# Ghundi/fluid_simulation

Hardware: AMD Instinct MI355X
Metric: cells_steps_per_sec (higher is better)
Workload: dtype f32

## Files before the change

### fluid_simulation_amd/csrc/kernels.hip

```cpp
#include <hip/hip_runtime.h>
#include "kernels.h"
#include "kernels_dev.h"
#include <type_traits>

namespace fs {

template <class T, int RY>
struct PlaneIn {
    T core[RY][4];
    T hb[4], ht[4];
    T eL[RY], eR[RY];
};
template <class T, int RY>
struct AuxIn {
    T rhs[RY][4];
    unsigned fl[RY];
};

template <class T, int RY, int ABL, bool PUSH>
__global__ __launch_bounds__(256) void jacobi_sweep_kernel(GridDesc g, SlabCtx sc, const T* __restrict__ src,
                                                            const T* __restrict__ rhs, T* __restrict__ dst,
                                                            const uint8_t* __restrict__ flags, int b, T a, T inv_c,
                                                            int z_first, int z_last, int zc_len, int z_stride, int nxw,
                                                            int nybg, int nblk, PeerPush pp)
// ... 774 lines not shown
    }
}


template <class T>
__global__ void bounds_faces_kernel(GridDesc g, SlabCtx sc, T* q, int b)
{
    const int W = g.W, H = g.H, D = g.D;
    const long nx = (long)H * D, ny = (long)W * D, nz = (long)W * H;
    for (long t = blockIdx.x * (long)blockDim.x + threadIdx.x; t < nx + ny + nz; t += (long)gridDim.x * blockDim.x) {
        if (t < nx) {
            int y = 1 + (int)(t % H), z = 1 + (int)(t / H);
            T in = q[cell(g, 1, y, z)];
            q[cell(g, 0, y, z)] = (b == 1) ? -in : in;
            q[cell(g, W + 1, y, z)] = q[cell(g, W, y, z)];
        } else if (t < nx + ny) {
            long u = t - nx;
            int x = 1 + (int)(u % W), z = 1 + (int)(u / W);
            T lo = q[cell(g, x, 1, z)], hi = q[cell(g, x, H, z)];
            q[cell(g, x, 0, z)] = (b == 2) ? -lo : lo;
            q[cell(g, x, H + 1, z)] = (b == 2) ? -hi : hi;
        } else {
            long u = t - nx - ny;
            int x = 1 + (int)(u % W), y = 1 + (int)(u / W);
            if (sc.lo_wall) {
                T lo = q[cell(g, x, y, 1)];
                q[cell(g, x, y, 0)] = (b == 3) ? -lo : lo;
            }
            if (sc.hi_wall) {
                T hi = q[cell(g, x, y, D)];
                q[cell(g, x, y, D + 1)] = (b == 3) ? -hi : hi;
            }
        }
    }
}

template <class T>
__global__ void bounds_zero_kernel(GridDesc g, T* q, const uint8_t* flags, int b)
{
    const int x = 1 + blockIdx.x * blockDim.x + threadIdx.x;
    const int y = 1 + blockIdx.y * blockDim.y + threadIdx.y;
    const int z = 1 + blockIdx.z;
    if (x > g.W || y > g.H) return;
    const unsigned zero_bits = (b == 0) ? F_SOLID : (F_SOLID | F_NEAR);
    long c = cell(g, x, y, z);
    if (flags[c] & zero_bits) q[c] = (T)0;
}

static inline dim3 cell_grid(const GridDesc& g) { return dim3((g.W + 63) / 64, (g.H + 3) / 4, g.D); }
static inline dim3 cell_block() { return dim3(64, 4, 1); }

template <class T>
void launch_set_bounds(hipStream_t st, const GridDesc& g, const SlabCtx& sc, T* q, const uint8_t* flags, int b)
{
    long faces = (long)g.H * g.D + (long)g.W * g.D + (long)g.W * g.H;
    int nb = (int)((faces + 255) / 256);
    if (nb > 4096) nb = 4096;
    hipLaunchKernelGGL((bounds_faces_kernel<T>), dim3(nb), dim3(256), 0, st, g, sc, q, b);
    hipLaunchKernelGGL((bounds_zero_kernel<T>), cell_grid(g), cell_block(), 0, st, g, q, flags, b);
}
template void launch_set_bounds<float>(hipStream_t, const GridDesc&, const SlabCtx&, float*, const uint8_t*, int);
template void launch_set_bounds<double>(hipStream_t, const GridDesc&, const SlabCtx&, double*, const uint8_t*, int);


template <class T, bool STORE_P>
__global__ __launch_bounds__(256) void divergence_kernel(GridDesc g, SlabCtx sc, const T* __restrict__ vx,
                                                          const T* __restrict__ vy, const T* __restrict__ vz,
                                                          T* __restrict__ dv, T* __restrict__ p,
                                                          const uint8_t* __restrict__ flags, T mhalf_h)
{
    const int x = 1 + blockIdx.x * blockDim.x + threadIdx.x;
    const int y = 1 + blockIdx.y * blockDim.y + threadIdx.y;
    const int z = 1 + blockIdx.z;
    if (x > g.W || y > g.H) return;
    const long c = cell(g, x, y, z);
    const unsigned f = flags[c];
    T d = (T)0;
    if (!(f & F_SOLID)) {
        T acc = (T)0;
        if (f & F_XP) acc += vx[c + 1];
        if (f & F_XM) acc -= vx[c - 1];
        if (f & F_YP) acc += vy[c + g.sy];
        if (f & F_YM) acc -= vy[c - g.sy];
        if (f & F_ZP) acc += vz[c + g.sz];
        if (f & F_ZM) acc -= vz[c - g.sz];
        d = mhalf_h * acc;
    }
    dv[c] = d;
    write_face_ghosts(g, sc, dv, c, x, y, z, d, 0);
    if constexpr (STORE_P) {
        p[c] = (T)0;
        write_face_ghosts(g, sc, p, c, x, y, z, (T)0, 0);
    }
}

template <class T>
void launch_divergence(hipStream_t st, const SweepTune& tune, const GridDesc& g, const SlabCtx& sc, const T* vx, const T* vy,
                       const T* vz, T* div, T* p, const uint8_t* flags, T mhalf_h, bool store_p)
{
    if (tune.project_cell) {
        if (store_p)
            hipLaunchKernelGGL((divergence_kernel<T, true>), cell_grid(g), cell_block(), 0, st, g, sc, vx, vy, vz, div, p, flags,
                               mhalf_h);
        else
            hipLaunchKernelGGL((divergence_kernel<T, false>), cell_grid(g), cell_block(), 0, st, g, sc, vx, vy, vz, div, p, flags,
                               mhalf_h);
        return;
    }
    constexpr int RY = 2;
    const MarchLaunch m = march_launch(g, RY);
    if (store_p)
        hipLaunchKernelGGL((divergence_march_kernel<T, RY, true>), dim3(m.nblk), dim3(256), 0, st, g, sc, vx, vy, vz, div, p, flags,
                           mhalf_h, m.zc_len, m.nxw, m.nybg, m.nblk);
    else
        hipLaunchKernelGGL((divergence_march_kernel<T, RY, false>), dim3(m.nblk), dim3(256), 0, st, g, sc, vx, vy, vz, div, p, flags,
                           mhalf_h, m.zc_len, m.nxw, m.nybg, m.nblk);
}
template void launch_divergence<float>(hipStream_t, const SweepTune&, const GridDesc&, const SlabCtx&, const float*,
                                       const float*, const float*, float*, float*, const uint8_t*, float, bool);
template void launch_divergence<double>(hipStream_t, const SweepTune&, const GridDesc&, const SlabCtx&, const double*,
                                        const double*, const double*, double*, double*, const uint8_t*, double, bool);

template <class T>
__device__ __forceinline__ T one_sided_grad(bool fp, bool fm, T pp, T pc, T pm, T h, T two_h)
{
    if (fp && fm) return (pp - pm) / two_h;
    if (fp) return (pp - pc) / h;
    if (fm) return (pc - pm) / h;
    return (T)0;
}

template <class T>
__global__ __launch_bounds__(256) void gradient_kernel(GridDesc g, SlabCtx sc, const T* __restrict__ p,
                                                        T* __restrict__ vx, T* __restrict__ vy, T* __restrict__ vz,
                                                        const uint8_t* __restrict__ flags, T h, T two_h)
{
    const int x = 1 + blockIdx.x * blockDim.x + threadIdx.x;
    const int y = 1 + blockIdx.y * blockDim.y + threadIdx.y;
    const int z = 1 + blockIdx.z;
    if (x > g.W || y > g.H) return;
    const long c = cell(g, x, y, z);
    const unsigned f = flags[c];
    T ux = vx[c], uy = vy[c], uz = vz[c];
    if (!(f & F_SOLID)) {
        const T pc = p[c];
        ux -= one_sided_grad<T>(f & F_XP, f & F_XM, p[c + 1], pc, p[c - 1], h, two_h);
        uy -= one_sided_grad<T>(f & F_YP, f & F_YM, p[c + g.sy], pc, p[c - g.sy], h, two_h);
        uz -= one_sided_grad<T>(f & F_ZP, f & F_ZM, p[c + g.sz], pc, p[c - g.sz], h, two_h);
    }
    const bool kill = (f & (F_SOLID | F_NEAR)) != 0;
    vx[c] = kill ? (T)0 : ux;
    vy[c] = kill ? (T)0 : uy;
    vz[c] = kill ? (T)0 : uz;
    write_face_ghosts(g, sc, vx, c, x, y, z, ux, 1);
    write_face_ghosts(g, sc, vy, c, x, y, z, uy, 2);
    write_face_ghosts(g, sc, vz, c, x, y, z, uz, 3);
}

template <class T>
void launch_gradient(hipStream_t st, const SweepTune& tune, const GridDesc& g, const SlabCtx& sc, const T* p, T* vx, T* vy,
                     T* vz, const uint8_t* flags, T h, T two_h)
{
    if (tune.project_cell) {
        hipLaunchKernelGGL((gradient_kernel<T>), cell_grid(g), cell_block(), 0, st, g, sc, p, vx, vy, vz, flags, h, two_h);
        return;
    }
    constexpr int RY = 2;
    const MarchLaunch m = march_launch(g, RY);
    hipLaunchKernelGGL((gradient_march_kernel<T, RY>), dim3(m.nblk), dim3(256), 0, st, g, sc, p, vx, vy, vz, flags, h, two_h,
                       m.zc_len, m.nxw, m.nybg, m.nblk);
}
template void launch_gradient<float>(hipStream_t, const SweepTune&, const GridDesc&, const SlabCtx&, const float*, float*,
                                     float*, float*, const uint8_t*, float, float);
template void launch_gradient<double>(hipStream_t, const SweepTune&, const GridDesc&, const SlabCtx&, const double*,
                                      double*, double*, double*, const uint8_t*, double, double);

template <class T>
__device__ __forceinline__ T clamp_ref(T v, T lo, T hi) { return (v < lo) ? lo : ((hi < v) ? hi : v); }

typedef float pair_f __attribute__((ext_vector_type(2), aligned(4)));
typedef double pair_d __attribute__((ext_vector_type(2), aligned(8)));
template <class T> struct PairOf;
template <> struct PairOf<float> { using type = pair_f; };
template <> struct PairOf<double> { using type = pair_d; };
template <class T>
__device__ __forceinline__ typename PairOf<T>::type ld_pair(const T* p) { return *reinterpret_cast<const typename PairOf<T>::type*>(p); }

template <class T>
__device__ __forceinline__ T back_trace_tab(const GridDesc& g, const SlabCtx& sc, const T* __restrict__ src, long zshift,
                                            const T* __restrict__ tab, int x, int y, int z, T ux, T uy, T uz, T kx, T ky, T kz);

template <class T, bool TAB>
__global__ __launch_bounds__(256) void advect_kernel(GridDesc g, SlabCtx sc, int b, T* __restrict__ field,
                                                      const T* __restrict__ prev, const T* vx, const T* vy,
                                                      const T* vz, const uint8_t* __restrict__ flags, T kx, T ky, T kz,
                                                      long prev_zshift, const T* __restrict__ tab)
{
    const int x = 1 + blockIdx.x * blockDim.x + threadIdx.x;
    const int y = 1 + blockIdx.y * blockDim.y + __builtin_amdgcn_readfirstlane(threadIdx.y);
    const int z = 1 + blockIdx.z;
    if (x > g.W || y > g.H) return;
    const long c = cell(g, x, y, z);
    const unsigned f = flags[c];
    const T one = (T)1, half = (T)0.5;
    T u = (T)0;
    if (!(f & F_SOLID)) {
        T ux, uy, uz;
        if (b == 0) {
            ux = vx[c]; uy = vy[c]; uz = vz[c];
        } else {
            const T own = prev[c + prev_zshift];
            ux = (b == 1) ? own : vx[c];
            uy = (b == 2) ? own : vy[c];
            uz = (b == 3) ? own : vz[c];
        }
        if constexpr (TAB) {
            u = back_trace_tab<T>(g, sc, prev, prev_zshift, tab, x, y, z, ux, uy, uz, kx, ky, kz);
        } else {
        const int zg = z + sc.zoff;
        T px = clamp_ref<T>((T)x - kx * ux, half, (T)g.W + half);
        T py = clamp_ref<T>((T)y - ky * uy, half, (T)g.H + half);
        T pz = clamp_ref<T>((T)zg - kz * uz, half, (T)sc.Dglobal + half);
        const int x0 = (int)floor(px), y0 = (int)floor(py), z0 = (int)floor(pz);
        const T tx = px - (T)x0, ty = py - (T)y0, tz = pz - (T)z0;
        const T* s = prev + prev_zshift + cell(g, x0, y0, z0 - sc.zoff);
        const auto q00 = ld_pair(s), q01 = ld_pair(s + g.sz), q10 = ld_pair(s + g.sy), q11 = ld_pair(s + g.sy + g.sz);
        const T a00 = q00.x * (one - tx) + q00.y * tx;
        const T a01 = q01.x * (one - tx) + q01.y * tx;
        const T a10 = q10.x * (one - tx) + q10.y * tx;
        const T a11 = q11.x * (one - tx) + q11.y * tx;
        const T b0 = a00 * (one - ty) + a10 * ty;
        const T b1 = a01 * (one - ty) + a11 * ty;
        u = b0 * (one - tz) + b1 * tz;
        }
    }
    const bool kill = (b != 0) && (f & F_NEAR);
    field[c] = kill ? (T)0 : u;
    write_face_ghosts(g, sc, field, c, x, y, z, u, b);
}

template <class T>
__device__ __forceinline__ T back_trace(const GridDesc& g, const SlabCtx& sc, const T* __restrict__ src, long zshift,
                                        int x, int y, int z, T ux, T uy, T uz, T kx, T ky, T kz)
{
    const T one = (T)1, half = (T)0.5;
    T px = clamp_ref<T>((T)x - kx * ux, half, (T)g.W + half);
    T py = clamp_ref<T>((T)y - ky * uy, half, (T)g.H + half);
    T pz = clamp_ref<T>((T)(z + sc.zoff) - kz * uz, half, (T)sc.Dglobal + half);
    const int x0 = (int)floor(px), y0 = (int)floor(py), z0 = (int)floor(pz);
    const T tx = px - (T)x0, ty = py - (T)y0, tz = pz - (T)z0;
    const T* s = src + zshift + cell(g, x0, y0, z0 - sc.zoff);
    const auto q00 = ld_pair(s), q01 = ld_pair(s + g.sz), q10 = ld_pair(s + g.sy), q11 = ld_pair(s + g.sy + g.sz);
    const T a00 = q00.x * (one - tx) + q00.y * tx;
    const T a01 = q01.x * (one - tx) + q01.y * tx;
    const T a10 = q10.x * (one - tx) + q10.y * tx;
    const T a11 = q11.x * (one - tx) + q11.y * tx;
    const T b0 = a00 * (one - ty) + a10 * ty;
    const T b1 = a01 * (one - ty) + a11 * ty;
    return b0 * (one - tz) + b1 * tz;
}

template <class T, bool TAB>
__global__ __launch_bounds__(256) void advect_velocity_kernel(GridDesc g, SlabCtx sc, T* __restrict__ vx,
                                                               T* __restrict__ vy, T* __restrict__ vz,
                                                               const T* __restrict__ px, const T* __restrict__ py,
                                                               const T* __restrict__ pz,
                                                               const uint8_t* __restrict__ flags, T kx, T ky, T kz,
                                                               long zshift, const T* __restrict__ tab)
{
    const int x = 1 + blockIdx.x * blockDim.x + threadIdx.x;
    const int y = 1 + blockIdx.y * blockDim.y + __builtin_amdgcn_readfirstlane(threadIdx.y);
    const int z = 1 + blockIdx.z;
    if (x > g.W || y > g.H) return;
    const long c = cell(g, x, y, z);
    const unsigned f = flags[c];
    const bool near = (f & F_NEAR) != 0;
    T nx = (T)0, ny = (T)0, nz = (T)0;
    T sx = (T)0, sy = (T)0;
    if (!(f & F_SOLID)) {
        const T oy = vy[c], oz = vz[c];
        if constexpr (TAB) {
            const long plane2 = 2 * (long)(g.H + 2) * (g.D + 2);
            nx = back_trace_tab<T>(g, sc, px, zshift, tab, x, y, z, px[c + zshift], oy, oz, kx, ky, kz);
            sx = near ? (T)0 : nx;
            ny = back_trace_tab<T>(g, sc, py, zshift, tab + plane2, x, y, z, sx, py[c + zshift], oz, kx, ky, kz);
            sy = near ? (T)0 : ny;
            nz = back_trace_tab<T>(g, sc, pz, zshift, tab + 2 * plane2, x, y, z, sx, sy, pz[c + zshift], kx, ky, kz);
        } else {
            nx = back_trace<T>(g, sc, px, zshift, x, y, z, px[c + zshift], oy, oz, kx, ky, kz);
            sx = near ? (T)0 : nx;
            ny = back_trace<T>(g, sc, py, zshift, x, y, z, sx, py[c + zshift], oz, kx, ky, kz);
            sy = near ? (T)0 : ny;
            nz = back_trace<T>(g, sc, pz, zshift, x, y, z, sx, sy, pz[c + zshift], kx, ky, kz);
        }
    }
    vx[c] = near ? (T)0 : nx;
    vy[c] = near ? (T)0 : ny;
    vz[c] = near ? (T)0 : nz;
    write_face_ghosts(g, sc, vx, c, x, y, z, nx, 1);
    write_face_ghosts(g, sc, vy, c, x, y, z, ny, 2);
    write_face_ghosts(g, sc, vz, c, x, y, z, nz, 3);
}

template <class T>
__global__ __launch_bounds__(256) void gradient_advect_velocity_kernel(GridDesc g, SlabCtx sc, const T* __restrict__ p,
                                                                        T* __restrict__ vx, T* __restrict__ vy,
                                                                        T* __restrict__ vz, const T* __restrict__ px,
                                                                        const T* __restrict__ py, const T* __restrict__ pz,
                                                                        const uint8_t* __restrict__ flags, T h, T two_h, T kx,
                                                                        T ky, T kz)
{
    const int x = 1 + blockIdx.x * blockDim.x + threadIdx.x;
    const int y = 1 + blockIdx.y * blockDim.y + __builtin_amdgcn_readfirstlane(threadIdx.y);
    const int z = 1 + blockIdx.z;
    if (x > g.W || y > g.H) return;
    const long c = cell(g, x, y, z);
    const unsigned f = flags[c];
    const bool near = (f & F_NEAR) != 0;
    T nx = (T)0, ny = (T)0, nz = (T)0;
    T sx = (T)0, sy = (T)0;
    if (!(f & F_SOLID)) {
        T oy = vy[c], oz = vz[c];
        const T pc = p[c];
        oy -= one_sided_grad<T>(f & F_YP, f & F_YM, p[c + g.sy], pc, p[c - g.sy], h, two_h);
        oz -= one_sided_grad<T>(f & F_ZP, f & F_ZM, p[c + g.sz], pc, p[c - g.sz], h, two_h);
        if (near) oy = oz = (T)0;
        nx = back_trace<T>(g, sc, px, 0, x, y, z, px[c], oy, oz, kx, ky, kz);
        sx = near ? (T)0 : nx;
        ny = back_trace<T>(g, sc, py, 0, x, y, z, sx, py[c], oz, kx, ky, kz);
        sy = near ? (T)0 : ny;
        nz = back_trace<T>(g, sc, pz, 0, x, y, z, sx, sy, pz[c], kx, ky, kz);
    }
    vx[c] = near ? (T)0 : nx;
    vy[c] = near ? (T)0 : ny;
    vz[c] = near ? (T)0 : nz;
    write_face_ghosts(g, sc, vx, c, x, y, z, nx, 1);
    write_face_ghosts(g, sc, vy, c, x, y, z, ny, 2);
    write_face_ghosts(g, sc, vz, c, x, y, z, nz, 3);
}

template <class T>
__global__ __launch_bounds__(256) void advect_columns_kernel(GridDesc g, const T* __restrict__ p0, const T* __restrict__ p1,
                                                              const T* __restrict__ p2, int nsrc, T* __restrict__ tab)
{
    const long plane = (long)(g.H + 2) * (g.D + 2);
    const long i = blockIdx.x * (long)blockDim.x + threadIdx.x;
    if (i >= plane) return;
    const int y = (int)(i % (g.H + 2)), z = (int)(i / (g.H + 2));
    const T one = (T)1, half = (T)0.5;
    for (int k = 0; k < nsrc; ++k) {
        const T* s = (k == 0 ? p0 : k == 1 ? p1 : p2) + cell(g, 0, y, z);
        tab[(2 * k + 0) * plane + i] = s[0] * (one - half) + s[1] * half;
        tab[(2 * k + 1) * plane + i] = s[g.W] * (one - half) + s[g.W + 1] * half;
    }
}

template <class T>
__device__ __forceinline__ T back_trace_tab(const GridDesc& g, const SlabCtx& sc, const T* __restrict__ src, long zshift,
                                            const T* __restrict__ tab, int x, int y, int z, T ux, T uy, T uz, T kx, T ky, T kz)
{
    const T one = (T)1, half = (T)0.5;
    const T px = clamp_ref<T>((T)x - kx * ux, half, (T)g.W + half);
    const T py = clamp_ref<T>((T)y - ky * uy, half, (T)g.H + half);
    const T pz = clamp_ref<T>((T)(z + sc.zoff) - kz * uz, half, (T)sc.Dglobal + half);
    const int y0 = (int)floor(py), z0 = (int)floor(pz);
    const T ty = py - (T)y0, tz = pz - (T)z0;
    T a00, a01, a10, a11;
    const bool lo = (px == half), hi = (px == (T)g.W + half);
    if (tab != nullptr && (lo || hi)) {
        const long plane = (long)(g.H + 2) * (g.D + 2);
        const T* t = tab + (hi ? plane : 0) + y0 + (long)z0 * (g.H + 2);
        a00 = t[0];
        a10 = t[1];
        a01 = t[g.H + 2];
        a11 = t[g.H + 3];
    } else {
        const int x0 = (int)floor(px);
        const T tx = px - (T)x0;
        const T* s = src + zshift + cell(g, x0, y0, z0 - sc.zoff);
        const auto q00 = ld_pair(s), q01 = ld_pair(s + g.sz), q10 = ld_pair(s + g.sy), q11 = ld_pair(s + g.sy + g.sz);
        a00 = q00.x * (one - tx) + q00.y * tx;
        a01 = q01.x * (one - tx) + q01.y * tx;
        a10 = q10.x * (one - tx) + q10.y * tx;
        a11 = q11.x * (one - tx) + q11.y * tx;
    }
    const T b0 = a00 * (one - ty) + a10 * ty;
    const T b1 = a01 * (one - ty) + a11 * ty;
    return b0 * (one - tz) + b1 * tz;
}

template <class T>
__global__ __launch_bounds__(256) void advect_row_kernel(GridDesc g, SlabCtx sc, int b, T* __restrict__ field,
                                                          const T* __restrict__ prev, const T* vx, const T* vy, const T* vz,
                                                          const uint8_t* __restrict__ kill, const T* __restrict__ tab, T kx,
                                                          T ky, T kz, long zshift)
{
    const int x0 = 1 + (blockIdx.x * 64 + (threadIdx.x & 63)) * 4;
    const int y = 1 + blockIdx.y * 4 + __builtin_amdgcn_readfirstlane(threadIdx.x >> 6);
    const int z = 1 + blockIdx.z;
    if (x0 > g.W || y > g.H) return;
    const long c = cell(g, x0, y, z);
    const unsigned kb = kill[(c + 3) >> 2];
    T own[4], ax[4], ay[4], az[4], u[4];
    ld_row(prev + c + zshift, b != 0, own);
    ld_row(vx + c, b != 1, ax);
    ld_row(vy + c, b != 2, ay);
    ld_row(vz + c, b != 3, az);
#pragma unroll
    for (int e = 0; e < 4; ++e) {
        u[e] = (T)0;
        if (x0 + e <= g.W && !((kb >> e) & 1u)) {
            const T ux = (b == 1) ? own[e] : ax[e];
            const T uy = (b == 2) ? own[e] : ay[e];
            const T uz = (b == 3) ? own[e] : az[e];
            u[e] = back_trace_tab<T>(g, sc, prev, zshift, tab, x0 + e, y, z, ux, uy, uz, kx, ky, kz);
        }
    }
    store_row_bounds<T>(g, sc, field, c, x0, y, z, u, (b == 0) ? (kb & 15u) : (kb >> 4), b);
}

template <class T>
__global__ __launch_bounds__(256) void advect_velocity_row_kernel(GridDesc g, SlabCtx sc, T* __restrict__ vx, T* __restrict__ vy,
                                                                   T* __restrict__ vz, const T* __restrict__ px,
                                                                   const T* __restrict__ py, const T* __restrict__ pz,
                                                                   const uint8_t* __restrict__ kill, const T* __restrict__ tab,
                                                                   T kx, T ky, T kz, long zshift)
{
    const int x0 = 1 + (blockIdx.x * 64 + (threadIdx.x & 63)) * 4;
    const int y = 1 + blockIdx.y * 4 + __builtin_amdgcn_readfirstlane(threadIdx.x >> 6);
    const int z = 1 + blockIdx.z;
    if (x0 > g.W || y > g.H) return;
    const long c = cell(g, x0, y, z);
    const unsigned kb = kill[(c + 3) >> 2];
    const unsigned near4 = kb >> 4;
    const long plane2 = 2 * (long)(g.H + 2) * (g.D + 2);
    const T* tx_ = tab, *ty_ = tab ? tab + plane2 : nullptr, *tz_ = tab ? tab + 2 * plane2 : nullptr;
    T ox[4], oy[4], oz[4], qy[4], qz[4], nx[4], ny[4], nz[4];
    ld_row(px + c + zshift, true, ox);
    ld_row(py + c + zshift, true, qy);
    ld_row(pz + c + zshift, true, qz);
    ld_row(vy + c, true, oy);
    ld_row(vz + c, true, oz);
#pragma unroll
    for (int e = 0; e < 4; ++e) {
        nx[e] = ny[e] = nz[e] = (T)0;
        if (x0 + e <= g.W && !((kb >> e) & 1u)) {
            const bool near = ((near4 >> e) & 1u) != 0;
            nx[e] = back_trace_tab<T>(g, sc, px, zshift, tx_, x0 + e, y, z, ox[e], oy[e], oz[e], kx, ky, kz);
            const T sx = near ? (T)0 : nx[e];
            ny[e] = back_trace_tab<T>(g, sc, py, zshift, ty_, x0 + e, y, z, sx, qy[e], oz[e], kx, ky, kz);
            const T sy = near ? (T)0 : ny[e];
            nz[e] = back_trace_tab<T>(g, sc, pz, zshift, tz_, x0 + e, y, z, sx, sy, qz[e], kx, ky, kz);
        }
    }
    store_row_bounds<T>(g, sc, vx, c, x0, y, z, nx, near4, 1);
    store_row_bounds<T>(g, sc, vy, c, x0, y, z, ny, near4, 2);
    store_row_bounds<T>(g, sc, vz, c, x0, y, z, nz, near4, 3);
}

template <class T, int NF>
__global__ __launch_bounds__(1024) void advect_tile_kernel(GridDesc g, SlabCtx sc, int b, T* __restrict__ f0, T* __restrict__ f1,
                                                            T* __restrict__ f2, const T* __restrict__ p0, const T* __restrict__ p1,
                                                            const T* __restrict__ p2, const T* vx, const T* vy, const T* vz,
                                                            const uint8_t* __restrict__ flags, T kx, T ky, T kz,
                                                            const T* __restrict__ tab, int R)
{
    constexpr int TY = 8, TZ = 8;
    extern __shared__ unsigned char win_raw[];
    T* win = reinterpret_cast<T*>(win_raw);
    const int ty0 = 1 + blockIdx.x * TY, tz0 = 1 + blockIdx.y * TZ;
    const int wy0 = max(0, ty0 - R), wy1 = min(g.H + 1, ty0 + TY + R), wz0 = max(0, tz0 - R), wz1 = min(g.D + 1, tz0 + TZ + R);
    const int WY = wy1 - wy0 + 1, WZ = wz1 - wz0 + 1;
    const long tplane = (long)(g.H + 2) * (g.D + 2);
    for (int k = 0; k < NF; ++k) {
        const T* t = tab + 2 * k * tplane;
        for (int i = threadIdx.x; i < WY * WZ; i += 1024) {
            const int yy = i % WY, zz = i / WY;
            win[(long)k * WY * WZ + i] = t[(wy0 + yy) + (long)(wz0 + zz) * (g.H + 2)];
        }
    }
    __syncthreads();
    const int lane = threadIdx.x & 63, wave = __builtin_amdgcn_readfirstlane(threadIdx.x >> 6);
    const T one = (T)1, half = (T)0.5;
    auto trace = [&](int k, const T* src, int x, int y, int z, T ux, T uy, T uz) -> T {
        const T px = clamp_ref<T>((T)x - kx * ux, half, (T)g.W + half);
        const T py = clamp_ref<T>((T)y - ky * uy, half, (T)g.H + half);
        const T pz = clamp_ref<T>((T)z - kz * uz, half, (T)g.D + half);
        const int y0 = (int)floor(py), z0 = (int)floor(pz);
        if (px == half && y0 >= wy0 && y0 + 1 <= wy1 && z0 >= wz0 && z0 + 1 <= wz1) {
            const T ty = py - (T)y0, tz = pz - (T)z0;
            const T* w = win + (long)k * WY * WZ + (y0 - wy0) + (long)(z0 - wz0) * WY;
            const T a00 = w[0], a10 = w[1], a01 = w[WY], a11 = w[WY + 1];
            const T b0 = a00 * (one - ty) + a10 * ty;
            const T b1 = a01 * (one - ty) + a11 * ty;
            return b0 * (one - tz) + b1 * tz;
        }
        return back_trace_tab<T>(g, sc, src, 0, tab + 2 * k * tplane, x, y, z, ux, uy, uz, kx, ky, kz);
    };
    for (int row = wave; row < TY * TZ; row += 16) {
        const int y = ty0 + row % TY, z = tz0 + row / TY;
        if (y > g.H || z > g.D) continue;
        for (int x = 1 + lane; x <= g.W; x += 64) {
            const long c = cell(g, x, y, z);
            const unsigned f = flags[c];
            const bool near = (f & F_NEAR) != 0;
            if constexpr (NF == 1) {
                T u = (T)0;
                if (!(f & F_SOLID)) {
                    T ux, uy, uz;
                    if (b == 0) {
                        ux = vx[c]; uy = vy[c]; uz = vz[c];
                    } else {
                        const T own = p0[c];
                        ux = (b == 1) ? own : vx[c];
                        uy = (b == 2) ? own : vy[c];
                        uz = (b == 3) ? own : vz[c];
                    }
                    u = trace(0, p0, x, y, z, ux, uy, uz);
                }
                f0[c] = ((b != 0) && near) ? (T)0 : u;
                write_face_ghosts(g, sc, f0, c, x, y, z, u, b);
            } else {
                T nx = (T)0, ny = (T)0, nz = (T)0;
                if (!(f & F_SOLID)) {
                    const T oy = f1[c], oz = f2[c];
                    nx = trace(0, p0, x, y, z, p0[c], oy, oz);
                    const T sx = near ? (T)0 : nx;
                    ny = trace(1, p1, x, y, z, sx, p1[c], oz);
                    const T sy = near ? (T)0 : ny;
                    nz = trace(2, p2, x, y, z, sx, sy, p2[c]);
                }
                f0[c] = near ? (T)0 : nx;
                f1[c] = near ? (T)0 : ny;
                f2[c] = near ? (T)0 : nz;
                write_face_ghosts(g, sc, f0, c, x, y, z, nx, 1);
                write_face_ghosts(g, sc, f1, c, x, y, z, ny, 2);
                write_face_ghosts(g, sc, f2, c, x, y, z, nz, 3);
            }
        }
    }
}

template <class T>
static int tile_window(int want, int nf)
{
    int r = want < 1 ? 1 : want;
    while (r > 1 && (long)nf * (8 + 2 * r + 1) * (8 + 2 * r + 1) * (long)sizeof(T) > 64 * 1024) --r;
    return r;
}

static inline dim3 row_grid(const GridDesc& g) { return dim3((g.W + 255) / 256, (g.H + 3) / 4, g.D); }

template <class T>
static const T* build_columns(hipStream_t st, const GridDesc& g, const SlabCtx& sc, const T* p0, const T* p1, const T* p2,
                              int nsrc, T* coltab, long zshift)
{
    if (!coltab || zshift != 0 || !(sc.lo_wall && sc.hi_wall)) return nullptr;
    const long plane = (long)(g.H + 2) * (g.D + 2);
    hipLaunchKernelGGL((advect_columns_kernel<T>), dim3((unsigned)((plane + 255) / 256)), dim3(256), 0, st, g, p0, p1, p2, nsrc,
                       coltab);
    return coltab;
}

template <class T>
void launch_advect_velocity(hipStream_t st, const SweepTune& tune, const GridDesc& g, const SlabCtx& sc, T* vx, T* vy, T* vz,
                            const T* px, const T* py, const T* pz, const uint8_t* flags, const uint8_t* kill, T* coltab, T kx,
                            T ky, T kz, long zshift)
{
    const T* tab = (tune.advect_cell == 1) ? nullptr : build_columns<T>(st, g, sc, px, py, pz, 3, coltab, zshift);
    if (tune.advect_cell == 3 && tab) {
        const int R = tile_window<T>(tune.advect_window, 3);
        const size_t lds = (size_t)3 * (8 + 2 * R + 1) * (8 + 2 * R + 1) * sizeof(T);
        hipLaunchKernelGGL((advect_tile_kernel<T, 3>), dim3((g.H + 7) / 8, (g.D + 7) / 8), dim3(1024), lds, st, g, sc, 0, vx, vy, vz, px,
                           py, pz, vx, vy, vz, flags, kx, ky, kz, tab, R);
        return;
    }
    if (tune.advect_cell) {
        if (tab)
            hipLaunchKernelGGL((advect_velocity_kernel<T, true>), cell_grid(g), cell_block(), 0, st, g, sc, vx, vy, vz, px, py,
                               pz, flags, kx, ky, kz, zshift, tab);
        else
            hipLaunchKernelGGL((advect_velocity_kernel<T, false>), cell_grid(g), cell_block(), 0, st, g, sc, vx, vy, vz, px, py,
                               pz, flags, kx, ky, kz, zshift, tab);
        return;
    }
    hipLaunchKernelGGL((advect_velocity_row_kernel<T>), row_grid(g), dim3(256), 0, st, g, sc, vx, vy, vz, px, py, pz, kill, tab,
                       kx, ky, kz, zshift);
}
template void launch_advect_velocity<float>(hipStream_t, const SweepTune&, const GridDesc&, const SlabCtx&, float*, float*,
                                            float*, const float*, const float*, const float*, const uint8_t*, const uint8_t*,
                                            float*, float, float, float, long);
template void launch_advect_velocity<double>(hipStream_t, const SweepTune&, const GridDesc&, const SlabCtx&, double*, double*,
                                             double*, const double*, const double*, const double*, const uint8_t*,
                                             const uint8_t*, double*, double, double, double, long);

template <class T>
void launch_gradient_advect_velocity(hipStream_t st, const GridDesc& g, const SlabCtx& sc, const T* p, T* vx, T* vy, T* vz,
                                     const T* px, const T* py, const T* pz, const uint8_t* flags, T h, T two_h, T kx, T ky, T kz)
{
    hipLaunchKernelGGL((gradient_advect_velocity_kernel<T>), cell_grid(g), cell_block(), 0, st, g, sc, p, vx, vy, vz, px, py, pz,
                       flags, h, two_h, kx, ky, kz);
}
template void launch_gradient_advect_velocity<float>(hipStream_t, const GridDesc&, const SlabCtx&, const float*, float*, float*,
                                                     float*, const float*, const float*, const float*, const uint8_t*, float,
                                                     float, float, float, float);
template void launch_gradient_advect_velocity<double>(hipStream_t, const GridDesc&, const SlabCtx&, const double*, double*, double*,
                                                      double*, const double*, const double*, const double*, const uint8_t*,
                                                      double, double, double, double, double);

template <class T>
void launch_advect(hipStream_t st, const SweepTune& tune, const GridDesc& g, const SlabCtx& sc, int b, T* field, const T* prev,
                   const T* vx, const T* vy, const T* vz, const uint8_t* flags, const uint8_t* kill, T* coltab, T kx, T ky, T kz,
                   long prev_zshift)
{
    const T* tab = (tune.advect_cell == 1) ? nullptr : build_columns<T>(st, g, sc, prev, prev, prev, 1, coltab, prev_zshift);
    if (tune.advect_cell == 3 && tab) {
        const int R = tile_window<T>(tune.advect_window, 1);
        const size_t lds = (size_t)(8 + 2 * R + 1) * (8 + 2 * R + 1) * sizeof(T);
        hipLaunchKernelGGL((advect_tile_kernel<T, 1>), dim3((g.H + 7) / 8, (g.D + 7) / 8), dim3(1024), lds, st, g, sc, b, field, field,
                           field, prev, prev, prev, vx, vy, vz, flags, kx, ky, kz, tab, R);
        return;
    }
    if (tune.advect_cell) {
        if (tab)
            hipLaunchKernelGGL((advect_kernel<T, true>), cell_grid(g), cell_block(), 0, st, g, sc, b, field, prev, vx, vy, vz,
                               flags, kx, ky, kz, prev_zshift, tab);
        else
            hipLaunchKernelGGL((advect_kernel<T, false>), cell_grid(g), cell_block(), 0, st, g, sc, b, field, prev, vx, vy, vz,
                               flags, kx, ky, kz, prev_zshift, tab);
        return;
    }
    hipLaunchKernelGGL((advect_row_kernel<T>), row_grid(g), dim3(256), 0, st, g, sc, b, field, prev, vx, vy, vz, kill, tab, kx,
                       ky, kz, prev_zshift);
}
template void launch_advect<float>(hipStream_t, const SweepTune&, const GridDesc&, const SlabCtx&, int, float*, const float*,
                                   const float*, const float*, const float*, const uint8_t*, const uint8_t*, float*, float, float,
                                   float, long);
template void launch_advect<double>(hipStream_t, const SweepTune&, const GridDesc&, const SlabCtx&, int, double*, const double*,
                                    const double*, const double*, const double*, const uint8_t*, const uint8_t*, double*, double,
                                    double, double, long);

template <class T>
__global__ void build_flags_kernel(GridDesc g, SlabCtx sc, const T* __restrict__ obs, uint8_t* __restrict__ flags,
                                   int zlo)
{
    const int x = 1 + blockIdx.x * blockDim.x + threadIdx.x;
    const int y = 1 + blockIdx.y * blockDim.y + threadIdx.y;
    const int z = zlo + blockIdx.z;
    if (x > g.W || y > g.H) return;
    const long c = cell(g, x, y, z);
    const int zg = z + sc.zoff;
    const bool rxp = x + 1 <= g.W, rxm = x - 1 >= 1, ryp = y + 1 <= g.H, rym = y - 1 >= 1;
    const bool rzp = zg + 1 <= sc.Dglobal, rzm = zg - 1 >= 1;
    const T one = (T)1, zero = (T)0;
    unsigned f = 0;
    if (obs[c] == one) {
        f = F_SOLID;
    } else {
        bool near = (rxp && obs[c + 1] == one) || (rxm && obs[c - 1] == one) || (ryp && obs[c + g.sy] == one) ||
                    (rym && obs[c - g.sy] == one) || (rzp && obs[c + g.sz] == one) || (rzm && obs[c - g.sz] == one);
        if (near) f |= F_NEAR;
    }
    if (rxp && obs[c + 1] == zero) f |= F_XP;
    if (rxm && obs[c - 1] == zero) f |= F_XM;
    if (ryp && obs[c + g.sy] == zero) f |= F_YP;
    if (rym && obs[c - g.sy] == zero) f |= F_YM;
    if (rzp && obs[c + g.sz] == zero) f |= F_ZP;
    if (rzm && obs[c - g.sz] == zero) f |= F_ZM;
    flags[c] = (uint8_t)f;
}

template <class T>
void launch_build_flags(hipStream_t st, const GridDesc& g, const SlabCtx& sc, const T* obs, uint8_t* flags)
{
    const int zlo = (g.zh >= 2 && !sc.lo_wall) ? 2 - g.zh : 1, zhi = (g.zh >= 2 && !sc.hi_wall) ? g.D + g.zh - 1 : g.D;
    dim3 grid = cell_grid(g);
    grid.z = zhi - zlo + 1;
    hipLaunchKernelGGL((build_flags_kernel<T>), grid, cell_block(), 0, st, g, sc, obs, flags, zlo);
}
template void launch_build_flags<float>(hipStream_t, const GridDesc&, const SlabCtx&, const float*, uint8_t*);
template void launch_build_flags<double>(hipStream_t, const GridDesc&, const SlabCtx&, const double*, uint8_t*);

__global__ void build_kill_kernel(GridDesc g, const uint8_t* __restrict__ flags, uint8_t* __restrict__ kill, int zlo)
{
    const int gx = blockIdx.x * blockDim.x + threadIdx.x;
    const int y = 1 + blockIdx.y * blockDim.y + threadIdx.y;
    const int z = zlo + blockIdx.z;
    const int x0 = 1 + 4 * gx;
    if (x0 > g.W || y > g.H) return;
    const long c = cell(g, x0, y, z);
    const unsigned f = *reinterpret_cast<const unsigned*>(flags + c);
    unsigned out = 0;
#pragma unroll
    for (int e = 0; e < 4; ++e) {
        const unsigned fe = (f >> (8 * e)) & 0xffu;
        if (fe & F_SOLID) out |= 1u << e;
        if (fe & (F_SOLID | F_NEAR)) out |= 16u << e;
    }
    kill[(c + 3) >> 2] = (uint8_t)out;
}
void launch_build_kill(hipStream_t st, const GridDesc& g, const SlabCtx& sc, const uint8_t* flags, uint8_t* kill)
{
    const int zlo = (g.zh >= 2 && !sc.lo_wall) ? 2 - g.zh : 1, zhi = (g.zh >= 2 && !sc.hi_wall) ? g.D + g.zh - 1 : g.D;
    const int ng = (g.W + 3) / 4;
    hipLaunchKernelGGL(build_kill_kernel, dim3((ng + 63) / 64, (g.H + 3) / 4, zhi - zlo + 1), dim3(64, 4, 1), 0, st, g,
                       flags, kill, zlo);
}

__global__ void build_clean_kernel(GridDesc g, const uint8_t* __restrict__ kill, uint32_t* __restrict__ tab, int words)
{
    __shared__ uint32_t w[64];
    const int z = blockIdx.x, lane = threadIdx.x & 63, wave = threadIdx.x >> 6;
    for (int i = threadIdx.x; i < words; i += blockDim.x) w[i] = 0u;
    __syncthreads();
    const int ng = (g.W + 3) / 4;
    for (int y = wave; y <= g.H + 1; y += blockDim.x / 64) {
        bool dirty = false;
        for (int gx = lane; gx < ng; gx += 64) dirty |= kill[(cell(g, 1 + 4 * gx, y, z) + 3) >> 2] != 0;
        if (__builtin_amdgcn_ballot_w64(dirty) == 0 && lane == 0) atomicOr(&w[y >> 5], 1u << (y & 31));
    }
    __syncthreads();
    for (int i = threadIdx.x; i < words; i += blockDim.x) tab[(long)z * words + i] = w[i];
}
void launch_build_clean(hipStream_t st, const GridDesc& g, const uint8_t* kill, uint32_t* tab, int words)
{
    hipLaunchKernelGGL(build_clean_kernel, dim3(g.D + 2), dim3(256), 0, st, g, kill, tab, words);
}

template <class T>
__global__ void inlet_velocity_kernel(GridDesc g, T* vx, T* vy, T* vz, T speed, int zlo)
{
    const int y = 1 + blockIdx.x * blockDim.x + threadIdx.x;
    const int z = zlo + blockIdx.y;
    if (y > g.H) return;
    const long c = cell(g, 1, y, z);
    vx[c] = speed;
    vy[c] = (T)0;
    vz[c] = (T)0;
}
template <class T>
__global__ void inlet_density_kernel(GridDesc g, T* dens, T amount, int zlo)
{
    const int y = 1 + blockIdx.x * blockDim.x + threadIdx.x;
    const int z = zlo + blockIdx.y;
    if (y > g.H) return;
    dens[cell(g, 1, y, z)] += amount;
}
template <class T>
void launch_inlet_velocity(hipStream_t st, const GridDesc& g, const SlabCtx& sc, T* vx, T* vy, T* vz, T speed)
{
    const int zlo = sc.lo_wall ? 1 : 1 - g.zh, zhi = sc.hi_wall ? g.D : g.D + g.zh;
    hipLaunchKernelGGL((inlet_velocity_kernel<T>), dim3((g.H + 63) / 64, zhi - zlo + 1), dim3(64), 0, st, g, vx, vy, vz,
                       speed, zlo);
}
template <class T>
void launch_inlet_density(hipStream_t st, const GridDesc& g, const SlabCtx& sc, T* dens, T amount)
{
    const int zlo = sc.lo_wall ? 1 : 1 - g.zh, zhi = sc.hi_wall ? g.D : g.D + g.zh;
    hipLaunchKernelGGL((inlet_density_kernel<T>), dim3((g.H + 63) / 64, zhi - zlo + 1), dim3(64), 0, st, g, dens, amount,
                       zlo);
}
template void launch_inlet_velocity<float>(hipStream_t, const GridDesc&, const SlabCtx&, float*, float*, float*, float);
template void launch_inlet_velocity<double>(hipStream_t, const GridDesc&, const SlabCtx&, double*, double*, double*, double);
template void launch_inlet_density<float>(hipStream_t, const GridDesc&, const SlabCtx&, float*, float);
template void launch_inlet_density<double>(hipStream_t, const GridDesc&, const SlabCtx&, double*, double);

template <class T, class U>
__global__ void pack_kernel(GridDesc g, const T* __restrict__ f, U* __restrict__ dense, int zlo)
{
    const int x = blockIdx.x * blockDim.x + threadIdx.x;
    const int y = blockIdx.y * blockDim.y + threadIdx.y;
    const int z = zlo + blockIdx.z;
    if (x > g.W + 1 || y > g.H + 1) return;
    dense[(long)x + (long)y * (g.W + 2) + (long)(z - zlo) * (g.W + 2) * (g.H + 2)] = (U)f[cell(g, x, y, z)];
}
template <class T, class U>
__global__ void unpack_kernel(GridDesc g, const U* __restrict__ dense, T* __restrict__ f, int zlo)
{
    const int x = blockIdx.x * blockDim.x + threadIdx.x;
    const int y = blockIdx.y * blockDim.y + threadIdx.y;
    const int z = zlo + blockIdx.z;
    if (x > g.W + 1 || y > g.H + 1) return;
    f[cell(g, x, y, z)] = (T)dense[(long)x + (long)y * (g.W + 2) + (long)(z - zlo) * (g.W + 2) * (g.H + 2)];
}
template <class T, class U>
void launch_pack(hipStream_t st, const GridDesc& g, const T* field, U* dense, int zlo, int zhi)
{
    if (zhi < zlo) return;
    hipLaunchKernelGGL((pack_kernel<T, U>), dim3((g.W + 2 + 63) / 64, (g.H + 2 + 3) / 4, zhi - zlo + 1), dim3(64, 4, 1),
                       0, st, g, field, dense, zlo);
}
template <class T, class U>
void launch_unpack(hipStream_t st, const GridDesc& g, const U* dense, T* field, int zlo, int zhi)
{
    if (zhi < zlo) return;
    hipLaunchKernelGGL((unpack_kernel<T, U>), dim3((g.W + 2 + 63) / 64, (g.H + 2 + 3) / 4, zhi - zlo + 1),
                       dim3(64, 4, 1), 0, st, g, dense, field, zlo);
}
#define FS_INST_PACK(T, U)                                                                     \
    template void launch_pack<T, U>(hipStream_t, const GridDesc&, const T*, U*, int, int);     \
    template void launch_unpack<T, U>(hipStream_t, const GridDesc&, const U*, T*, int, int);
FS_INST_PACK(float, float)
FS_INST_PACK(float, double)
FS_INST_PACK(double, float)
FS_INST_PACK(double, double)
FS_INST_PACK(float, uint8_t)
FS_INST_PACK(double, uint8_t)

template <class T>
__global__ void copy_kernel(const T* __restrict__ src, T* __restrict__ dst, long n4)
{
    for (long i = blockIdx.x * (long)blockDim.x + threadIdx.x; i < n4; i += (long)gridDim.x * blockDim.x)
        reinterpret_cast<V4<T>*>(dst)[i] = reinterpret_cast<const V4<T>*>(src)[i];
}
template <class T>
void launch_copy(hipStream_t st, const GridDesc& g, const T* src, T* dst)
{
    long n4 = g.n / 4;
    hipLaunchKernelGGL((copy_kernel<T>), dim3(2048), dim3(256), 0, st, src - g.lead, dst - g.lead, n4);
}
template void launch_copy<float>(hipStream_t, const GridDesc&, const float*, float*);
template void launch_copy<double>(hipStream_t, const GridDesc&, const double*, double*);

template <class T>
__global__ __launch_bounds__(256) void stats_partial_kernel(GridDesc g, const T* __restrict__ f, double* part, int zlo,
                                                             int zhi)
{
    const long rows = (long)(g.H + 2) * (zhi - zlo + 1);
    double s = 0.0, mn = 1e300, mx = -1e300;
    for (long r = blockIdx.x; r < rows; r += gridDim.x) {
        int y = (int)(r % (g.H + 2)), z = zlo + (int)(r / (g.H + 2));
        for (int x = threadIdx.x; x <= g.W + 1; x += blockDim.x) {
            double v = (double)f[cell(g, x, y, z)];
            s += v;
            mn = v < mn ? v : mn;
            mx = v > mx ? v : mx;
        }
    }
    __shared__ double sh[3][256];
    sh[0][threadIdx.x] = s; sh[1][threadIdx.x] = mn; sh[2][threadIdx.x] = mx;
    __syncthreads();
    for (int k = 128; k > 0; k >>= 1) {
        if ((int)threadIdx.x < k) {
            sh[0][threadIdx.x] += sh[0][threadIdx.x + k];
            sh[1][threadIdx.x] = fmin(sh[1][threadIdx.x], sh[1][threadIdx.x + k]);
            sh[2][threadIdx.x] = fmax(sh[2][threadIdx.x], sh[2][threadIdx.x + k]);
        }
        __syncthreads();
    }
    if (threadIdx.x == 0) {
        part[3 * blockIdx.x + 0] = sh[0][0];
        part[3 * blockIdx.x + 1] = sh[1][0];
        part[3 * blockIdx.x + 2] = sh[2][0];
    }
}
__global__ void stats_final_kernel(const double* part, int n, double* out3)
{
    if (threadIdx.x != 0 || blockIdx.x != 0) return;
    double s = 0.0, mn = 1e300, mx = -1e300;
    for (int i = 0; i < n; ++i) {
        s += part[3 * i];
        mn = fmin(mn, part[3 * i + 1]);
        mx = fmax(mx, part[3 * i + 2]);
    }
    out3[0] = s; out3[1] = mn; out3[2] = mx;
}
template <class T>
void launch_stats(hipStream_t st, const GridDesc& g, const T* field, double* out3, double* scratch, int nscratch,
                  int zlo, int zhi)
{
    int nb = nscratch / 3;
    if (nb > 1024) nb = 1024;
    hipLaunchKernelGGL((stats_partial_kernel<T>), dim3(nb), dim3(256), 0, st, g, field, scratch, zlo, zhi);
    hipLaunchKernelGGL(stats_final_kernel, dim3(1), dim3(64), 0, st, scratch, nb, out3);
}
template void launch_stats<float>(hipStream_t, const GridDesc&, const float*, double*, double*, int, int, int);
template void launch_stats<double>(hipStream_t, const GridDesc&, const double*, double*, double*, int, int, int);

template <class T>
__global__ void point_kernel(T* p, long idx, T amount, int set_instead)
{
    if (threadIdx.x == 0 && blockIdx.x == 0) p[idx] = set_instead ? amount : p[idx] + amount;
}
template <class T>
void launch_point_add(hipStream_t st, T* p, long idx, T amount, int set_instead)
{
    hipLaunchKernelGGL((point_kernel<T>), dim3(1), dim3(64), 0, st, p, idx, amount, set_instead);
}
template void launch_point_add<float>(hipStream_t, float*, long, float, int);
template void launch_point_add<double>(hipStream_t, double*, long, double, int);

}
```

### fluid_simulation_amd/csrc/kernels_dev.h

```cpp
#pragma once
#include <hip/hip_runtime.h>
#include "kernels.h"

namespace fs {

template <class T>
struct alignas(16) V4 {
    T e[4];
};

__device__ __forceinline__ long cell(const GridDesc& g, int x, int y, int z)
{
    return (long)x + (long)y * g.sy + (long)z * g.sz;
}

template <class T>
__device__ __forceinline__ void write_face_ghosts(const GridDesc& g, const SlabCtx& sc, T* q, long c, int x, int y,
                                                  int z, T u, int b)
{
    if (x == 1) q[c - 1] = (b == 1) ? -u : u;
    if (x == g.W) q[c + 1] = u;
    if (y == 1) q[c - g.sy] = (b == 2) ? -u : u;
    if (y == g.H) q[c + g.sy] = (b == 2) ? -u : u;
    if (z == 1 && sc.lo_wall) q[c - g.sz] = (b == 3) ? -u : u;
    if (z == g.D && sc.hi_wall) q[c + g.sz] = (b == 3) ? -u : u;
}

template <bool PUSH, class V>
__device__ __forceinline__ void put(V* p, const V& v, long dl, long dh)
{
    *p = v;
    if constexpr (PUSH) {
        if (dl) *reinterpret_cast<V*>(reinterpret_cast<char*>(p) + dl) = v;
        if (dh) *reinterpret_cast<V*>(reinterpret_cast<char*>(p) + dh) = v;
    }
}

__device__ __forceinline__ int xcd_contiguous(int b, int nblk)
{
    int q = nblk >> 3, r = nblk & 7, k = b & 7;
    return k * q + (k < r ? k : r) + (b >> 3);
}

template <class T>
struct MarchTile {
    int lane, x0, y0, zbeg, zend;
    bool lane_on, full_group, edge_l, edge_r, live;
    long row0;
};
template <class T, int RY>
__device__ __forceinline__ MarchTile<T> march_tile(const GridDesc& g, int zc_len, int nxw, int nybg, int nblk)
{
    MarchTile<T> t;
    const int v = xcd_contiguous(blockIdx.x, nblk);
    const int xw = v % nxw, ybg = (v / nxw) % nybg, zc = v / (nxw * nybg);
    t.lane = threadIdx.x & 63;
    t.y0 = 1 + (ybg * 4 + __builtin_amdgcn_readfirstlane(threadIdx.x >> 6)) * RY;
    t.x0 = 1 + xw * 256 + t.lane * 4;
    t.lane_on = t.x0 <= g.W;
    t.zbeg = 1 + zc * zc_len;
    t.zend = min(g.D, t.zbeg + zc_len - 1);
    t.full_group = (t.x0 + 3 <= g.W);
    t.edge_l = t.lane_on && (t.lane == 0);
    t.edge_r = t.lane_on && t.full_group && ((t.lane == 63) || (t.x0 + 4 > g.W));
    t.live = (t.y0 <= g.H) && (t.zbeg <= t.zend);
    t.row0 = cell(g, t.x0, t.y0, 0);
    return t;
}
template <class T>
__device__ __forceinline__ void ld_row(const T* ptr, bool on, T (&out)[4])
{
    V4<T> q = {{(T)0, (T)0, (T)0, (T)0}};
    if (on) q = *reinterpret_cast<const V4<T>*>(ptr);
#pragma unroll
    for (int e = 0; e < 4; ++e) out[e] = q.e[e];
}

struct MarchLaunch {
    int zc_len, nxw, nybg, nblk;
};
inline MarchLaunch march_launch(const GridDesc& g, int RY)
{
    MarchLaunch m;
    m.nxw = (g.W + 255) / 256;
    const int nyb = (g.H + RY - 1) / RY;
    m.nybg = (nyb + 3) / 4;
    const long per_layer = (long)m.nxw * m.nybg;
    long want = (2048 + per_layer - 1) / per_layer;
    if (want < 1) want = 1;
    m.zc_len = (int)((g.D + want - 1) / want);
    if (m.zc_len < 8) m.zc_len = g.D < 8 ? g.D : 8;
    const int nzc = (g.D + m.zc_len - 1) / m.zc_len;
    m.nblk = (int)(per_layer * nzc);
    return m;
}

}
```

Measured before the change: 2.150 billion.

## Remap gradient-advect blocks into y-bands walked along z with XCD-contiguous ordering

Replaces the 3D grid for the fused gradient+advect-velocity kernel with a 1D grid. Blocks are ordered so that each XCD walks y-bands sized to fit a cache budget of roughly 1 MiB across 7 arrays, marching along z. The aim is better L2/MALL reuse of neighbouring planes for the p gradient and the back-trace reads, using the XCD-contiguous assignment already used elsewhere. The costs are extra index arithmetic per thread, padded blocks that exit early, and a fallback to the old grid when the block count overflows.

```diff
diff --git a/fluid_simulation_amd/csrc/kernels.hip b/fluid_simulation_amd/csrc/kernels.hip
--- a/fluid_simulation_amd/csrc/kernels.hip
+++ b/fluid_simulation_amd/csrc/kernels.hip
@@ -1100,18 +1100,17 @@
     write_face_ghosts(g, sc, vz, c, x, y, z, nz, 3);
 }
 
-template <class T>
-__global__ __launch_bounds__(256) void gradient_advect_velocity_kernel(GridDesc g, SlabCtx sc, const T* __restrict__ p,
+template <class T, bool BANDS>
+__global__ __launch_bounds__(256) void gradient_advect_velocity_kernel(GridDesc g, SlabCtx sc, AdvectMap am,
+                                                                        const T* __restrict__ p,
                                                                         T* __restrict__ vx, T* __restrict__ vy,
                                                                         T* __restrict__ vz, const T* __restrict__ px,
                                                                         const T* __restrict__ py, const T* __restrict__ pz,
                                                                         const uint8_t* __restrict__ flags, T h, T two_h, T kx,
                                                                         T ky, T kz)
 {
-    const int x = 1 + blockIdx.x * blockDim.x + threadIdx.x;
-    const int y = 1 + blockIdx.y * blockDim.y + __builtin_amdgcn_readfirstlane(threadIdx.y);
-    const int z = 1 + blockIdx.z;
-    if (x > g.W || y > g.H) return;
+    int x, y, z;
+    if (!advect_thread_cell<BANDS>(g, am, x, y, z)) return;
     const long c = cell(g, x, y, z);
     const unsigned f = flags[c];
     const bool near = (f & F_NEAR) != 0;
@@ -1396,8 +1395,13 @@
 void launch_gradient_advect_velocity(hipStream_t st, const GridDesc& g, const SlabCtx& sc, const T* p, T* vx, T* vy, T* vz,
                                      const T* px, const T* py, const T* pz, const uint8_t* flags, T h, T two_h, T kx, T ky, T kz)
 {
-    hipLaunchKernelGGL((gradient_advect_velocity_kernel<T>), cell_grid(g), cell_block(), 0, st, g, sc, p, vx, vy, vz, px, py, pz,
-                       flags, h, two_h, kx, ky, kz);
+    const AdvectMap am = advect_map(g.W, g.H, g.D, g.sy * (long)sizeof(T));
+    if (am.nblk > 0)
+        hipLaunchKernelGGL((gradient_advect_velocity_kernel<T, true>), dim3((unsigned)am.nblk), cell_block(), 0, st, g, sc, am, p,
+                           vx, vy, vz, px, py, pz, flags, h, two_h, kx, ky, kz);
+    else
+        hipLaunchKernelGGL((gradient_advect_velocity_kernel<T, false>), cell_grid(g), cell_block(), 0, st, g, sc, am, p, vx, vy,
+                           vz, px, py, pz, flags, h, two_h, kx, ky, kz);
 }
 template void launch_gradient_advect_velocity<float>(hipStream_t, const GridDesc&, const SlabCtx&, const float*, float*, float*,
                                                      float*, const float*, const float*, const float*, const uint8_t*, float,
diff --git a/fluid_simulation_amd/csrc/kernels_dev.h b/fluid_simulation_amd/csrc/kernels_dev.h
--- a/fluid_simulation_amd/csrc/kernels_dev.h
+++ b/fluid_simulation_amd/csrc/kernels_dev.h
@@ -1,4 +1,66 @@
 #pragma once
+
+#if defined(__HIPCC__)
+#define FS_HD __host__ __device__
+#else
+#define FS_HD
+#endif
+
+namespace fs {
+
+FS_HD inline int xcd_contiguous(int b, int nblk)
+{
+    int q = nblk >> 3, r = nblk & 7, k = b & 7;
+    return k * q + (k < r ? k : r) + (b >> 3);
+}
+
+struct AdvectMap {
+    int nx, bh, walks, nblk;
+};
+constexpr long ADVECT_BAND_BYTES = 1L << 20;
+constexpr int ADVECT_BAND_ARRAYS = 7;
+
+FS_HD inline AdvectMap advect_map(int W, int H, int D, long row_bytes)
+{
+    AdvectMap m;
+    m.nx = (W + 63) / 64;
+    const int nyb = (H + 3) / 4;
+    long fit = ADVECT_BAND_BYTES / (ADVECT_BAND_ARRAYS * row_bytes) / 4;
+    if (fit < 1) fit = 1;
+    m.walks = (int)((nyb + 8 * fit - 1) / (8 * fit));
+    m.bh = (nyb + 8 * m.walks - 1) / (8 * m.walks);
+    const long n = 8L * m.walks * m.bh * m.nx * D;
+    m.nblk = n < (1L << 30) ? (int)n : 0;
+    return m;
+}
+
+FS_HD inline bool advect_map_block(const AdvectMap& m, int H, int D, int b, int* xt, int* yb, int* z)
+{
+    const int v = xcd_contiguous(b, m.nblk);
+    const int per_plane = m.bh * m.nx;
+    const int per_band = per_plane * D;
+    const int band = v / per_band;
+    const int i = v - band * per_band;
+    const int zz = i / per_plane, j = i - zz * per_plane;
+    const int yl = j / m.nx;
+    *xt = j - yl * m.nx;
+    *yb = band * m.bh + yl;
+    *z = 1 + zz;
+    return *yb * 4 < H;
+}
+
+FS_HD inline bool advect_map_cell(const AdvectMap& m, int W, int H, int D, int b, int tx, int ty, int* x, int* y, int* z)
+{
+    int xt, yb;
+    if (!advect_map_block(m, H, D, b, &xt, &yb, z)) return false;
+    *x = 1 + xt * 64 + tx;
+    *y = 1 + yb * 4 + ty;
+    return *x <= W && *y <= H;
+}
+
+}
+
+#if defined(__HIPCC__)
 #include <hip/hip_runtime.h>
 #include "kernels.h"
 
@@ -36,10 +98,15 @@
     }
 }
 
-__device__ __forceinline__ int xcd_contiguous(int b, int nblk)
+template <bool BANDS>
+__device__ __forceinline__ bool advect_thread_cell(const GridDesc& g, const AdvectMap& m, int& x, int& y, int& z)
 {
-    int q = nblk >> 3, r = nblk & 7, k = b & 7;
-    return k * q + (k < r ? k : r) + (b >> 3);
+    const int ty = __builtin_amdgcn_readfirstlane(threadIdx.y);
+    if constexpr (BANDS) return advect_map_cell(m, g.W, g.H, g.D, blockIdx.x, threadIdx.x, ty, &x, &y, &z);
+    x = 1 + blockIdx.x * 64 + threadIdx.x;
+    y = 1 + blockIdx.y * 4 + ty;
+    z = 1 + blockIdx.z;
+    return x <= g.W && y <= g.H;
 }
 
 template <class T>
@@ -96,3 +163,4 @@
 }
 
 }
+#endif
```

Measured after the change: 2.157 billion (median of 6 runs). No clear change (+0.3%).
